# Chang-Tun-Yu/HLS-final-Visual-Odometry

Measured on AMD Instinct MI355X. Metric: stereo frame-pairs/sec (detect+match), KITTI 1241x376; matches bit-exact, higher is better.
Workload: dtype u8; 1 GPU; KITTI 1241x376 stereo quad-match (prev/curr x L/R), default 50x50 bins; noise=0, gpu_max_hw_queues=4, streams_per_gpu=256, frames_in_hbm=8, parallelism=1x independent stream groups

## Files before the change

### hls-final-visual-odometry_amd/csrc/kernels_match.hip

```cpp
#include "vh_findmatch.h"
#include "vh_wave.h"
#include <algorithm>
#include <cstdlib>
#include <type_traits>

#ifdef VH_FLOW_STATS
__device__ unsigned long long g_flow_stats[12];
extern "C" int32_t vh_debug_flow_stats(unsigned long long *out, int32_t reset) {
  if (hipMemcpyFromSymbol(out, HIP_SYMBOL(g_flow_stats), sizeof(g_flow_stats)) != hipSuccess) return -3;
  if (reset) { unsigned long long z[12] = {0}; if (hipMemcpyToSymbol(HIP_SYMBOL(g_flow_stats), z, sizeof(z)) != hipSuccess) return -3; }
  return 0;
}
#define VH_STAT(k, n) do { if ((threadIdx.x & 63) == 0) atomicAdd(&g_flow_stats[k], (unsigned long long)(n)); } while (0)
#else
#define VH_STAT(k, n) do { } while (0)
#endif

#ifndef VH_MATCH_WAVES
#define VH_MATCH_WAVES 7
#endif

namespace {

template <bool MAX>
__device__ __forceinline__ int32_t row16_allreduce(int32_t v) {
#define VH_ROW_STEP(CTRL)                                                                   \
  {                                                                                         \
    const int32_t t = __builtin_amdgcn_update_dpp(v, v, CTRL, 0xF, 0xF, false);             \
    v = MAX ? max(v, t) : min(v, t);                                                        \
  }
  VH_ROW_STEP(0x128)
  VH_ROW_STEP(0x124)
  VH_ROW_STEP(0x122)
  VH_ROW_STEP(0x121)
#undef VH_ROW_STEP
  return v;
}

template <class T>
__device__ __forceinline__ T ld_off(const T *base, uint32_t byte_off) { return *(const T *)((const char *)base + byte_off); }
template <class T>
__device__ __forceinline__ void st_off(T *base, uint32_t byte_off, T x) { *(T *)((char *)base + byte_off) = x; }
template <class T>
__device__ __forceinline__ T ld_uniform(const T *p) { return *(const __attribute__((address_space(4))) T *)(uintptr_t)p; }
__device__ __forceinline__ int32_t ld_uniform_i32(const int32_t *p) { return __builtin_amdgcn_readfirstlane(ld_uniform(p)); }

template <bool TESTED, class First, class Step>
__device__ __forceinline__ void walk_columns(const VhSets &s, const int32_t *__restrict__ cbs, int32_t c, int32_t UB0, int32_t UB1, int32_t VB0,
                                             int32_t VB1, int32_t ULO_MAX, int32_t UHI_MIN, int32_t VA0, int32_t VA1, First first, Step step) {
  const int32_t lane = threadIdx.x & 63;
  const bool merged = !TESTED && VB0 == 0 && VB1 == s.vbn - 1;
  const int32_t UB1w = merged ? UB0 : UB1;
  for (int32_t cb = UB0; cb <= UB1w; cb += 64) {
    const int32_t ncb = min(64, UB1w - cb + 1);
    int32_t t_p0 = 0, t_p1 = 0, t_a0 = 0, t_a1 = 0;
    if (lane < ncb) {
      const int32_t row = (c * s.ubn + cb + lane) * s.vbn;
      t_p0 = ld_off(cbs, (uint32_t)(row + VB0) * 4u);
      t_p1 = ld_off(cbs, (uint32_t)(merged ? (c * s.ubn + UB1 + 1) * s.vbn : row + VB1 + 1) * 4u);
      if (TESTED) {
        const int32_t ubx = cb + lane;
        const bool in_ = ubx * s.binsize >= ULO_MAX && ubx * s.binsize + s.binsize - 1 <= UHI_MIN;
        t_a0 = in_ ? ((VA0 <= VA1) ? cbs[row + VA0] : t_p1) : 1;
        t_a1 = in_ ? ((VA0 <= VA1) ? cbs[row + VA1 + 1] : t_p1) : 0;
      }
    }
    int32_t ci = -1, pc = -64, p1 = 0;
    const auto advance = [&]() -> bool {
      pc += 64;
      while (pc >= p1) {
        if (++ci >= ncb) return false;
        pc = __builtin_amdgcn_readlane(t_p0, ci); p1 = __builtin_amdgcn_readlane(t_p1, ci);
      }
      return true;
    };
    if (!advance()) continue;
    first(pc, p1);
    for (;;) {
      const int32_t c_pc = pc, c_p1 = p1, c_ci = ci;
      const bool more = advance();
      int32_t pa0 = 1, pa1 = 0;
      if (TESTED) { pa0 = __builtin_amdgcn_readlane(t_a0, c_ci); pa1 = __builtin_amdgcn_readlane(t_a1, c_ci); }
      step(c_pc, c_p1, pa0, pa1, more, pc, p1);
      if (!more) break;
    }
  }
}

template <bool TESTED, bool NEED_UV, class Consume>
__device__ __forceinline__ void walk_region(const VhSets &s, const int32_t *__restrict__ cbs, const uint32_t *__restrict__ cuv,
                                            const uint4 *__restrict__ cdesc, int32_t c, int32_t UB0, int32_t UB1, int32_t VB0,
                                            int32_t VB1, int32_t ULO_MAX, int32_t UHI_MIN, int32_t VA0, int32_t VA1,
                                            Consume consume) {
  const int32_t lane = threadIdx.x & 63;
  int32_t pl = 0;
  uint32_t gu = 0;
  uint4 g0, g1;
  const auto load = [&](int32_t pc, int32_t p1) __attribute__((always_inline)) {
    pl = min(pc + lane, p1 - 1);
    if (NEED_UV) gu = cuv[pl];
    g0 = cdesc[2 * (int64_t)pl]; g1 = cdesc[2 * (int64_t)pl + 1];
  };
  walk_columns<TESTED>(s, cbs, c, UB0, UB1, VB0, VB1, ULO_MAX, UHI_MIN, VA0, VA1, load,
    [&](int32_t pc, int32_t p1, int32_t pa0, int32_t pa1, bool more, int32_t npc, int32_t np1) __attribute__((always_inline)) {
      const int32_t c_pl = pl;
      const uint32_t c_gu = gu;
      const uint4 c_g0 = g0, c_g1 = g1;
      if (more) load(npc, np1);
      consume(pc, p1, pa0, pa1, c_pl, c_gu, c_g0, c_g1);
    });
}

__device__ __forceinline__ void glds16(const void *gbase, uint32_t byte_off, uint32_t lds_dst) {
  asm volatile("s_mov_b32 m0, %2\n\ts_nop 0\n\tglobal_load_lds_dwordx4 %0, %1" ::"v"(byte_off), "s"(gbase), "s"(lds_dst) : "memory");
}
__device__ __forceinline__ void glds4(const void *gbase, uint32_t byte_off, uint32_t lds_dst) {
  asm volatile("s_mov_b32 m0, %2\n\ts_nop 0\n\tglobal_load_lds_dword %0, %1" ::"v"(byte_off), "s"(gbase), "s"(lds_dst) : "memory");
}
__device__ __forceinline__ uint32_t lds_addr(const void *p) {
  return __builtin_amdgcn_readfirstlane((uint32_t)(uintptr_t)(const __attribute__((address_space(3))) void *)p);
}

template <bool TESTED, class Consume>
__device__ __forceinline__ void walk_region_lds(const VhSets &s, const int32_t *__restrict__ cbs, const uint32_t *__restrict__ cuv,
                                                const uint4 *__restrict__ cdesc, int32_t c, int32_t UB0, int32_t UB1, int32_t VB0,
                                                int32_t VB1, int32_t ULO_MAX, int32_t UHI_MIN, int32_t VA0, int32_t VA1,
                                                uint4 *wD, uint32_t *wU, Consume consume) {
  const uint32_t ldsD = lds_addr(wD), ldsU = lds_addr(wU);
  const uint32_t lane32 = (uint32_t)(threadIdx.x & 63) * 32u;
  const auto issue = [&](int32_t b, int32_t pc, int32_t p1) __attribute__((always_inline)) {
    const uint32_t off = min((uint32_t)pc * 32u + lane32, (uint32_t)(p1 - 1) * 32u);
    glds16(cdesc, off, ldsD + (uint32_t)b * 2048u); glds16(cdesc, off + 16u, ldsD + (uint32_t)b * 2048u + 1024u);
    if (TESTED) glds4(cuv, off >> 3, ldsU + (uint32_t)b * 256u);
  };
  int32_t buf = 0;
  walk_columns<TESTED>(s, cbs, c, UB0, UB1, VB0, VB1, ULO_MAX, UHI_MIN, VA0, VA1,
    [&](int32_t pc, int32_t p1) __attribute__((always_inline)) {
      asm volatile("s_waitcnt lgkmcnt(0)" ::: "memory");
      buf = 0;
      issue(0, pc, p1);
    },
    [&](int32_t pc, int32_t p1, int32_t pa0, int32_t pa1, bool more, int32_t npc, int32_t np1) __attribute__((always_inline)) {
      const int32_t c_buf = buf;
      if (more) {
        buf ^= 1;
        asm volatile("s_waitcnt lgkmcnt(0)" ::: "memory");
        issue(buf, npc, np1);
        if (TESTED) asm volatile("s_waitcnt vmcnt(3)" ::: "memory");
        else asm volatile("s_waitcnt vmcnt(2)" ::: "memory");
      } else {
        asm volatile("s_waitcnt vmcnt(0)" ::: "memory");
      }
      consume(pc, p1, pa0, pa1, (const uint4 *)(wD + c_buf * 128), (const uint32_t *)(wU + c_buf * 64));
    });
}

__device__ __forceinline__ uint64_t tested_key_uniform_query(const uint32_t (&qd)[8], us2 lo2, us2 span2, uint32_t uv2,
                                                             const uint4 &b0, const uint4 &b1, uint32_t relpos) {
  const bool out = outside_window(uv2, lo2, span2);
  const uint32_t sad = sad32(make_uint4(qd[0], qd[1], qd[2], qd[3]), make_uint4(qd[4], qd[5], qd[6], qd[7]), b0, b1, 0);
  return out ? ~0ull : (((uint64_t)sad << 32) | relpos);
}

enum { KEY_HI16 = 0, KEY_W19 = 1, KEY_64 = 2 };
template <int KM> struct KeyT { typedef uint32_t type; };
template <> struct KeyT<KEY_64> { typedef uint64_t type; };
template <int KM>
__device__ __forceinline__ typename KeyT<KM>::type sad_key(const uint4 &a0, const uint4 &a1, const uint4 &b0, const uint4 &b1, uint32_t seed) {
  if (KM == KEY_HI16) return (typename KeyT<KM>::type)sad32<true>(a0, a1, b0, b1, seed);
  const uint32_t sad = sad32(a0, a1, b0, b1, 0);
  if (KM == KEY_W19) return (typename KeyT<KM>::type)((sad << 19) | seed);
  return (typename KeyT<KM>::type)(((uint64_t)sad << 32) | seed);
}
template <int KM>
__device__ __forceinline__ typename KeyT<KM>::type key_none_floor() {
  typedef typename KeyT<KM>::type key_t;
  return KM == KEY_HI16 ? (key_t)0xFFFF0000u : KM == KEY_W19 ? (key_t)0xFFF80000u : (key_t)0x0000FFFF00000000ull;
}
__device__ __forceinline__ int32_t key_mode_of(int32_t class_count, int32_t wide_keys) {
  if (class_count + 64 <= 0x10000 && !wide_keys) return KEY_HI16;
  return class_count <= VH_CLASS_POS_MAX && wide_keys < 2 ? KEY_W19 : KEY_64;
}

template <int Q, int P, int KM>
__device__ __forceinline__ int32_t join_phases(const typename KeyT<KM>::type (&best_key)[Q]) {
  static_assert(Q == 2 && P == 4, "the join splits the wave into two slots of two 16-lane rows");
  if (KM == KEY_64) {
    uint64_t k[Q];
#pragma unroll
    for (int32_t qi = 0; qi < Q; qi++) {
      k[qi] = (uint64_t)best_key[qi];
#pragma unroll
      for (int32_t d = 16; d < 64; d <<= 1) k[qi] = min(k[qi], vh_shfl_xor_u64(k[qi], d));
    }
    const uint64_t kk = (threadIdx.x & 32) ? k[1] : k[0];
    return kk >= key_none_floor<KEY_64>() ? -1 : (int32_t)(uint32_t)kk;
  }
  const auto h = __builtin_amdgcn_permlane32_swap((uint32_t)best_key[0], (uint32_t)best_key[1], false, false);
  const uint32_t kh = min(h[0], h[1]);
  const auto r = __builtin_amdgcn_permlane16_swap(kh, kh, false, false);
  const uint32_t k = min(r[0], r[1]);
  return k >= key_none_floor<KM>() ? -1 : (int32_t)(k & (KM == KEY_HI16 ? 0xFFFFu : 0x7FFFFu));
}

#ifndef VH_REDO_G
#define VH_REDO_G 2
#endif
struct RedoGroup {
  uint32_t qd[VH_REDO_G][8];
  us2 lo2[VH_REDO_G];
  int32_t lane[VH_REDO_G], n;
  int32_t umin, umax, vmin, vmax;
};
template <int Q>
__device__ __forceinline__ bool redo_take(uint64_t &todo, const uint4 (&a0)[Q], const uint4 (&a1)[Q], const uint32_t (&uv1)[Q],
                                          int32_t radius, int32_t rv, RedoGroup &g) {
  g.n = 0; g.umin = g.vmin = 0x7FFFFFFF; g.umax = g.vmax = -1;
#pragma unroll
  for (int32_t k = 0; k < VH_REDO_G; k++) {
    if (!todo) break;
    const int32_t fl = (int32_t)__builtin_ctzll(todo), fq = fl >> 5;
    todo &= todo - 1;
    uint4 x0 = a0[0], x1 = a1[0];
    uint32_t xu = uv1[0];
#pragma unroll
    for (int32_t qi = 1; qi < Q; qi++) if (fq == qi) { x0 = a0[qi]; x1 = a1[qi]; xu = uv1[qi]; }
    g.qd[k][0] = __builtin_amdgcn_readlane(x0.x, fl); g.qd[k][1] = __builtin_amdgcn_readlane(x0.y, fl);
    g.qd[k][2] = __builtin_amdgcn_readlane(x0.z, fl); g.qd[k][3] = __builtin_amdgcn_readlane(x0.w, fl);
    g.qd[k][4] = __builtin_amdgcn_readlane(x1.x, fl); g.qd[k][5] = __builtin_amdgcn_readlane(x1.y, fl);
    g.qd[k][6] = __builtin_amdgcn_readlane(x1.z, fl); g.qd[k][7] = __builtin_amdgcn_readlane(x1.w, fl);
    const uint32_t quv1 = __builtin_amdgcn_readlane(xu, fl);
    const int32_t u1 = (int32_t)(quv1 & 0xFFFF), v1 = (int32_t)(quv1 >> 16);
    g.lo2[k] = window_lo2(quv1, radius, rv);
    g.lane[k] = fl; g.n = k + 1;
    g.umin = min(g.umin, u1); g.umax = max(g.umax, u1); g.vmin = min(g.vmin, v1); g.vmax = max(g.vmax, v1);
  }
  return g.n > 0;
}

template <int Q> struct TileOut {
  int32_t wp;
  uint4 a0[Q], a1[Q];
  uint32_t uv1[Q];
  int32_t qpos[Q];
  bool valid[Q];
};

template <int Q, int P, bool SPEC, bool FLOW>
__device__ __forceinline__ void finish_tile(const VhSets &s, const VhMatchArgs &a, int32_t pass, int32_t stream, int32_t qset, int32_t cset,
                                            int32_t c, int32_t pbase, int32_t pcnt, const TileOut<Q> &o,
                                            int32_t *__restrict__ best, int32_t *__restrict__ redo_count) {
  static_assert(Q == 2 && P == 4, "one query per lane: slot lane >> 5, on the first 16-lane row of each half (join_phases)");
  const int32_t lane = threadIdx.x & 63;
  const uint32_t *__restrict__ cuv = s.s_uv + (int64_t)cset * s.cap;
  const uint4 *__restrict__ cdesc = (const uint4 *)(s.s_desc + (int64_t)cset * s.cap * 8);
  const int32_t *__restrict__ cbs = s.bin_start + (int64_t)cset * (s.nbins + 1);
  const int32_t rv = FLOW ? a.radius : a.disp_tol;
  const us2 span2 = window_span2(a.radius, rv);
  const int32_t *__restrict__ cidx = s.s_idx + (int64_t)cset * s.cap;
  const int32_t *__restrict__ qidx = s.s_idx + (int64_t)qset * s.cap;
  int32_t *__restrict__ tbl = best + ((int64_t)stream * 4 + a.pass[pass].slot) * s.cap;
  const bool hi = lane & 32;
  const bool mine = !(lane & 16) && (hi ? o.valid[1] : o.valid[0]);
  const uint32_t uv1 = hi ? o.uv1[1] : o.uv1[0];
  const int32_t qpos = hi ? o.qpos[1] : o.qpos[0];
  int32_t res = -1;
  bool fail = false;
  if (mine && o.wp >= 0) {
    int32_t wp = o.wp;
    VH_CHECK_RANGE(s, 7, wp, 0, pcnt);
    res = pbase + wp;
    if (SPEC) fail = outside_window(ld_off(cuv, (uint32_t)res * 4u), window_lo2(uv1, a.radius, rv), span2);
  }
  if (SPEC) {
    uint64_t todo = __ballot(fail);
    if (todo) {
      const int32_t nfail = (int32_t)__popcll(todo);
      VH_STAT(FLOW ? 7 : 10, nfail);
      if (lane == 0) atomicAdd(redo_count, nfail);
      RedoGroup g;
      while (redo_take<Q>(todo, o.a0, o.a1, o.uv1, a.radius, rv, g)) {
        uint64_t kk[VH_REDO_G];
#pragma unroll
        for (int32_t k = 0; k < VH_REDO_G; k++) kk[k] = ~0ull;
        if (FLOW) {
          const VhBins b = bins_of_interest(s, VhWindow{g.umin - a.radius, g.umax + a.radius, g.vmin - rv, g.vmax + rv});
          walk_region<false, true>(s, cbs, cuv, cdesc, c, b.ub0, b.ub1, b.vb0, b.vb1, 0, 0, 0, 0,
            [&](int32_t, int32_t, int32_t, int32_t, int32_t pl, uint32_t gu, const uint4 &g0, const uint4 &g1) {
#pragma unroll
              for (int32_t k = 0; k < VH_REDO_G; k++)
                if (k < g.n) kk[k] = min(kk[k], tested_key_uniform_query(g.qd[k], g.lo2[k], span2, gu, g0, g1, (uint32_t)(pl - pbase)));
            });
        } else {
          const int32_t *__restrict__ crs = s.row_start + (int64_t)cset * (4 * s.H + 1);
          const int32_t *__restrict__ cpos = s.r_pos + (int64_t)cset * s.cap;
          const int32_t x0 = ld_uniform_i32(crs + c * s.H + max(g.vmin - rv, 0));
          const int32_t x1 = ld_uniform_i32(crs + c * s.H + min(g.vmax + rv, s.H - 1) + 1);
          for (int32_t x = x0 + lane; x < x1; x += 64) {
            int32_t cp = cpos[x];
            VH_CHECK_RANGE(s, 3, cp, pbase, pbase + pcnt);
            const uint32_t gu = cuv[cp];
            const uint4 g0 = cdesc[2 * (int64_t)cp], g1 = cdesc[2 * (int64_t)cp + 1];
#pragma unroll
            for (int32_t k = 0; k < VH_REDO_G; k++)
              if (k < g.n) kk[k] = min(kk[k], tested_key_uniform_query(g.qd[k], g.lo2[k], span2, gu, g0, g1, (uint32_t)(cp - pbase)));
          }
        }
#pragma unroll
        for (int32_t k = 0; k < VH_REDO_G; k++)
          if (k < g.n) {
            const uint64_t kf = vh_wave_min_u64(kk[k]);
            int32_t wp = (int32_t)(uint32_t)kf;
            if (kf != ~0ull) VH_CHECK_RANGE(s, 7, wp, 0, pcnt);
            if (lane == g.lane[k]) res = kf == ~0ull ? -1 : pbase + wp;
          }
      }
    }
  }
  if (mine) st_off(tbl, (uint32_t)ld_off(qidx, (uint32_t)qpos * 4u) * 4u, res < 0 ? 0 : ld_off(cidx, (uint32_t)res * 4u));
}

struct FlowRegion {
  int32_t UB0, UB1, VB0, VB1;
  int32_t ULO_MAX, UHI_MIN, VA0, VA1;
};
template <int Q, int P, bool SPEC>
__device__ __forceinline__ FlowRegion flow_queries(const VhSets &s, const VhMatchArgs &a, int32_t rv, int32_t qset, int32_t q0, int32_t q1,
                                                   int32_t c, TileOut<Q> &out) {
  constexpr int L = 64 / P;
  static_assert(L == 8 || L == 16, "every 16-lane row must hold the whole tile (row-wise window reduction)");
  const int32_t l = (threadIdx.x & 63) % L;
  const uint32_t *__restrict__ quv = s.s_uv + (int64_t)qset * s.cap;
  const uint4 *__restrict__ qdesc = (const uint4 *)(s.s_desc + (int64_t)qset * s.cap * 8);
  bool (&valid)[Q] = out.valid;
  uint4 (&a0)[Q] = out.a0, (&a1)[Q] = out.a1;
  uint32_t (&uv1)[Q] = out.uv1;
  int32_t umin = 0x7FFFFFFF, umax = -1, vmin = 0x7FFFFFFF, vmax = -1;
  int32_t (&qp)[Q] = out.qpos;
  const int32_t *__restrict__ qsnake = s.snake_pos + (int64_t)qset * s.cap;
#pragma unroll
  for (int32_t qi = 0; qi < Q; qi++) {
    const int32_t q = q0 + L * qi + l;
    valid[qi] = q < q1;
    qp[qi] = valid[qi] ? q : q0;
    if (VH_SNAKE) qp[qi] = ld_off(qsnake, (uint32_t)qp[qi] * 4u);
#ifdef VH_CHECK
    {
      const int32_t *qbs = s.bin_start + (int64_t)qset * (s.nbins + 1);
      VH_CHECK_RANGE(s, 14, qp[qi], qbs[c * s.ubn * s.vbn], qbs[(c + 1) * s.ubn * s.vbn]);
    }
#endif
  }
#pragma unroll
  for (int32_t qi = 0; qi < Q; qi++) {
    const int32_t ql = qp[qi];
    uv1[qi] = ld_off(quv, (uint32_t)ql * 4u);
    a0[qi] = ld_off(qdesc, (uint32_t)ql * 32u); a1[qi] = ld_off(qdesc, (uint32_t)ql * 32u + 16u);
    const int32_t u1 = uv1[qi] & 0xFFFF, v1 = uv1[qi] >> 16;
    umin = min(umin, u1); umax = max(umax, u1); vmin = min(vmin, v1); vmax = max(vmax, v1);
  }
  umin = __builtin_amdgcn_readfirstlane(row16_allreduce<false>(umin));
  umax = __builtin_amdgcn_readfirstlane(row16_allreduce<true>(umax));
  vmin = __builtin_amdgcn_readfirstlane(row16_allreduce<false>(vmin));
  vmax = __builtin_amdgcn_readfirstlane(row16_allreduce<true>(vmax));
  const VhBins ub = bins_of_interest(s, VhWindow{umin - a.radius, umax + a.radius, vmin - rv, vmax + rv});
  FlowRegion r;
  r.UB0 = ub.ub0; r.UB1 = ub.ub1; r.VB0 = ub.vb0; r.VB1 = ub.vb1;
  r.ULO_MAX = umax - a.radius; r.UHI_MIN = umin + a.radius;
  const int32_t VLO_MAX = vmax - rv, VHI_MIN = vmin + rv;
  r.VA0 = SPEC ? 0 : max(r.VB0, (max(VLO_MAX, 0) + s.binsize - 1) / s.binsize);
  r.VA1 = SPEC ? 0 : min(r.VB1, (VHI_MIN + 1) / s.binsize - 1);
  VH_STAT(0, 1); VH_STAT(5, q1 - q0); VH_STAT(6, r.UB1 - r.UB0 + 1);
  return r;
}

template <int Q, int P, int KM, bool SPEC>
__device__ __forceinline__ void flow_tile(const VhSets &s, const VhMatchArgs &a, int32_t rv, int32_t cset, int32_t c, const FlowRegion &r,
                                          int32_t pbase, uint4 *wD, uint32_t *wU, TileOut<Q> &out) {
  constexpr int L = 64 / P;
  constexpr int TRIP = 2 * P;
  constexpr int CH = 64 / TRIP;
  static_assert(P * (2 * CH - 1) <= 64, "the chunk-local seeds P * k must be inline constants (integers up to 64)");
  const int32_t ph = (threadIdx.x & 63) / L;
  const uint32_t *__restrict__ cuv = s.s_uv + (int64_t)cset * s.cap;
  const uint4 *__restrict__ cdesc = (const uint4 *)(s.s_desc + (int64_t)cset * s.cap * 8);
  const int32_t *__restrict__ cbs = s.bin_start + (int64_t)cset * (s.nbins + 1);
  const uint4 (&a0)[Q] = out.a0, (&a1)[Q] = out.a1;
  typedef typename KeyT<KM>::type key_t;
  const key_t KNONE = (key_t)~(key_t)0;
  key_t best_key[Q];
  int32_t v_lo[Q];
  us2 lo2[Q];
#pragma unroll
  for (int32_t qi = 0; qi < Q; qi++) {
    v_lo[qi] = (int32_t)(out.uv1[qi] >> 16) - rv;
    lo2[qi] = window_lo2(out.uv1[qi], a.radius, rv);
    best_key[qi] = KNONE;
  }
  const us2 span2 = window_span2(a.radius, rv);

  constexpr uint32_t LNONE = 0xFFFF0000u;
  auto make_key = [&](auto test, int32_t qi, uint32_t uv2, const uint4 &b0, const uint4 &b1, uint32_t seed) -> uint32_t {
    constexpr int TEST = decltype(test)::value;
    bool out = false;
    if (TEST == 2) {
      out = outside_window(uv2, lo2[qi], span2);
    } else if (TEST == 1) {
      out = (uint32_t)((int32_t)(uv2 >> 16) - v_lo[qi]) > (uint32_t)(2 * rv);
    }
    const uint32_t key = sad_key<KEY_HI16>(a0[qi], a1[qi], b0, b1, seed);
    return (TEST != 0 && out) ? LNONE : key;
  };
  auto global_key = [](uint32_t k, uint32_t vbase) -> key_t {
    if (KM == KEY_HI16) return (key_t)(k + vbase);
    const uint32_t pos = (k & 0xFFFFu) + vbase;
    if (KM == KEY_W19) return (key_t)(((k & 0xFFFF0000u) << 3) | pos);
    return (key_t)(((uint64_t)(k >> 16) << 32) | pos);
  };
  walk_region_lds<!SPEC>(s, cbs, cuv, cdesc, c, r.UB0, r.UB1, r.VB0, r.VB1, r.ULO_MAX, r.UHI_MIN, r.VA0, r.VA1, wD, wU,
    [&](int32_t pc, int32_t p1, int32_t pa0, int32_t pa1, const uint4 *cD, const uint32_t *cU) {
      VH_STAT(1, 1);
      const int32_t mcnt = min(64, p1 - pc);
      const int32_t nt = (mcnt + TRIP - 1) / TRIP;
      const uint4 *rd = cD + ph;
      const uint32_t *ru = cU + ph;
      uint32_t cm[Q];
      auto trip = [&](auto test, int32_t t) __attribute__((always_inline)) {
        VH_STAT(2 + decltype(test)::value, 1);
        const int32_t o = TRIP * t;
        const uint4 dA0 = rd[o], dA1 = rd[o + 64], dB0 = rd[o + P], dB1 = rd[o + 64 + P];
        uint32_t uA = 0, uB = 0;
        if (decltype(test)::value != 0) { uA = ru[o]; uB = ru[o + P]; }
#pragma unroll
        for (int32_t qi = 0; qi < Q; qi++) {
          const uint32_t kA = make_key(test, qi, uA, dA0, dA1, (uint32_t)o), kB = make_key(test, qi, uB, dB0, dB1, (uint32_t)(o + P));
          cm[qi] = t == 0 ? min(kA, kB) : min(min(kA, kB), cm[qi]);
        }
      };
      if (SPEC && nt == CH) {
#pragma unroll
        for (int32_t t = 0; t < CH; t++) {
          trip(std::integral_constant<int, 0>{}, t);
          if (t & 1) __builtin_amdgcn_sched_barrier(0);
        }
      } else if (SPEC || pa0 > pa1) {
        constexpr int TEST = SPEC ? 0 : 2;
#pragma unroll
        for (int32_t t = 0; t < CH; t++) {
          if (t >= nt) break;
          trip(std::integral_constant<int, TEST>{}, t);
        }
      } else {
        const int32_t ta = min((min(max(pa0 - pc, 0), mcnt) + TRIP - 1) / TRIP, nt);
        const int32_t tb = max(min(max(pa1 - pc, 0), mcnt) / TRIP, ta);
#pragma unroll
        for (int32_t t = 0; t < CH; t++) {
          if (t >= nt) break;
          if (t >= ta && t < tb) trip(std::integral_constant<int, 0>{}, t);
          else trip(std::integral_constant<int, 1>{}, t);
        }
      }
      const uint32_t vbase = (uint32_t)(pc - pbase + ph);
#pragma unroll
      for (int32_t qi = 0; qi < Q; qi++) best_key[qi] = min(best_key[qi], global_key(cm[qi], vbase));
    });
  out.wp = join_phases<Q, P, KM>(best_key);
}

template <bool SPEC, bool FLOW, class Tile>
__device__ __forceinline__ void search_tile(const VhSets &s, const VhMatchArgs &a, int32_t pass, int32_t stream, int32_t qset, int32_t cset,
                                            int32_t c, int32_t *__restrict__ best, int32_t *__restrict__ redo_count,
                                            TileOut<VH_FLOW_Q> &out, Tile tile) {
  const int32_t *cbs = s.bin_start + (int64_t)cset * (s.nbins + 1);
  const int32_t pbase = ld_uniform_i32(cbs + c * s.ubn * s.vbn);
  const int32_t pend = ld_uniform_i32(cbs + (c + 1) * s.ubn * s.vbn);
  const int32_t km = key_mode_of(pend - pbase, a.wide_keys);
  if (km == KEY_HI16) tile(std::integral_constant<int, KEY_HI16>{}, pbase, pend - pbase);
  else if (km == KEY_W19) tile(std::integral_constant<int, KEY_W19>{}, pbase, pend - pbase);
  else tile(std::integral_constant<int, KEY_64>{}, pbase, pend - pbase);
  finish_tile<VH_FLOW_Q, VH_FLOW_P, SPEC, FLOW>(s, a, pass, stream, qset, cset, c, pbase, pend - pbase, out, best, redo_count);
}

template <bool SPEC>
__device__ __forceinline__ void flow_pass(const VhSets &s, const VhMatchArgs &a, int32_t pass, int32_t stream, int32_t qset,
                                          int32_t cset, uint4 *wD, uint32_t *wU, int32_t *__restrict__ best, int32_t *__restrict__ redo_count) {
  const int32_t ntile = ld_uniform_i32(s.tile_cnt + qset);
  for (int32_t tile = __builtin_amdgcn_readfirstlane(blockIdx.x * 4 + (threadIdx.x >> 6)); tile < ntile;
       tile += gridDim.x * 4) {
    typedef int32_t i32x4 __attribute__((ext_vector_type(4)));
    const i32x4 t = ld_uniform((const i32x4 *)(s.tiles + (int64_t)qset * s.max_tiles + tile));
    const int32_t q0 = __builtin_amdgcn_readfirstlane(t.x), q1 = __builtin_amdgcn_readfirstlane(t.y);
    const int32_t c = __builtin_amdgcn_readfirstlane(t.z);
    TileOut<VH_FLOW_Q> out;
    const int32_t rv = a.pass[pass].flow ? a.radius : a.disp_tol;
    const FlowRegion r = flow_queries<VH_FLOW_Q, VH_FLOW_P, SPEC>(s, a, rv, qset, q0, q1, c, out);
    search_tile<SPEC, true>(s, a, pass, stream, qset, cset, c, best, redo_count, out,
      [&](auto km, int32_t pbase, int32_t) __attribute__((always_inline)) {
        flow_tile<VH_FLOW_Q, VH_FLOW_P, decltype(km)::value, SPEC>(s, a, rv, cset, c, r, pbase, wD, wU, out);
      });
  }
}

template <int Q, int P, int KM, bool SPEC>
__device__ __forceinline__ void rows_tile(const VhSets &s, const VhMatchArgs &a, int32_t pass, int32_t stream, int32_t qset,
                                          int32_t cset, int32_t q0, int32_t q1, int32_t c, int32_t pbase, int32_t pcnt, uint4 *wD,
                                          uint32_t *wU, uint32_t *wV, TileOut<Q> &out) {
  constexpr int L = 64 / P;
  static_assert(L == 8 || L == 16, "every 16-lane row must hold the whole tile");
  constexpr int TRIP = 2 * P;
  const int32_t lane = threadIdx.x & 63, ph = lane / L, l = lane % L;
  const int32_t nrow = 4 * s.H;
  const int32_t *__restrict__ crs = s.row_start + (int64_t)cset * (nrow + 1);
  const int32_t *__restrict__ qpos = s.r_pos + (int64_t)qset * s.cap;
  const uint32_t *__restrict__ quv = s.s_uv + (int64_t)qset * s.cap;
  const uint4 *__restrict__ qdesc = (const uint4 *)(s.s_desc + (int64_t)qset * s.cap * 8);
  const int32_t *__restrict__ cpos = s.r_pos + (int64_t)cset * s.cap;
  const uint32_t *__restrict__ cuv = s.s_uv + (int64_t)cset * s.cap;
  const uint4 *__restrict__ cdesc = (const uint4 *)(s.s_desc + (int64_t)cset * s.cap * 8);

  bool (&valid)[Q] = out.valid;
  uint4 (&a0)[Q] = out.a0, (&a1)[Q] = out.a1;
  uint32_t (&uv1)[Q] = out.uv1;
  int32_t (&qp)[Q] = out.qpos;
  typedef typename KeyT<KM>::type key_t;
  key_t best_key[Q];
  us2 lo2[Q];
  const us2 span2 = window_span2(a.radius, a.disp_tol);
  int32_t vmin = 0x7FFFFFFF, vmax = -1;
#pragma unroll
  for (int32_t qi = 0; qi < Q; qi++) {
    const int32_t q = q0 + L * qi + l;
    valid[qi] = q < q1;
    qp[qi] = ld_off(qpos, (uint32_t)(valid[qi] ? q : q0) * 4u);
    VH_CHECK_RANGE(s, 1, qp[qi], 0, s.cap);
    uv1[qi] = ld_off(quv, (uint32_t)qp[qi] * 4u);
    a0[qi] = ld_off(qdesc, (uint32_t)qp[qi] * 32u); a1[qi] = ld_off(qdesc, (uint32_t)qp[qi] * 32u + 16u);
    const int32_t v1 = uv1[qi] >> 16;
    lo2[qi] = window_lo2(uv1[qi], a.radius, a.disp_tol);
    best_key[qi] = (key_t)~(key_t)0;
    vmin = min(vmin, v1); vmax = max(vmax, v1);
  }
  vmin = __builtin_amdgcn_readfirstlane(row16_allreduce<false>(vmin));
  vmax = __builtin_amdgcn_readfirstlane(row16_allreduce<true>(vmax));
  VH_STAT(8, 1); VH_STAT(11, q1 - q0);
  const int32_t VLO = max(vmin - a.disp_tol, 0), VHI = min(vmax + a.disp_tol, s.H - 1);
  const int32_t r0 = ld_uniform_i32(crs + c * s.H + VLO);
  const int32_t r1 = ld_uniform_i32(crs + c * s.H + VHI + 1);
  for (int32_t rc = r0; rc < r1; rc += 64) {
    const int32_t mcnt = min(64, r1 - rc);
    int32_t cp = ld_off(cpos, (uint32_t)min(rc + lane, r1 - 1) * 4u);
    VH_CHECK_RANGE(s, 2, cp, pbase, pbase + pcnt);
    const uint4 g0 = ld_off(cdesc, (uint32_t)cp * 32u), g1 = ld_off(cdesc, (uint32_t)cp * 32u + 16u);
    uint32_t gu = 0;
    if (!SPEC) gu = ld_off(cuv, (uint32_t)cp * 4u);
    asm volatile("s_waitcnt lgkmcnt(0)" ::: "memory");
    wD[lane] = g0; wD[64 + lane] = g1; wU[lane] = (uint32_t)(cp - pbase);
    if (!SPEC) wV[lane] = gu;
    asm volatile("s_waitcnt lgkmcnt(0)" ::: "memory");
    const int32_t jend = (mcnt + TRIP - 1) & ~(TRIP - 1);
    VH_STAT(9, jend / TRIP);
    const uint4 *rd = wD + ph;
    const uint32_t *ru = wU + ph, *rv = wV + ph;
    for (int32_t j = 0; j < jend; j += TRIP) {
      const uint4 dA0 = rd[0], dA1 = rd[64], dB0 = rd[P], dB1 = rd[64 + P];
      const uint32_t sA = ru[0], sB = ru[P];
      uint32_t uA = 0, uB = 0;
      if (!SPEC) { uA = rv[0]; uB = rv[P]; }
#pragma unroll
      for (int32_t qi = 0; qi < Q; qi++) {
        key_t kA = sad_key<KM>(a0[qi], a1[qi], dA0, dA1, sA), kB = sad_key<KM>(a0[qi], a1[qi], dB0, dB1, sB);
        if (!SPEC) {
          kA = outside_window(uA, lo2[qi], span2) ? (key_t)~(key_t)0 : kA;
          kB = outside_window(uB, lo2[qi], span2) ? (key_t)~(key_t)0 : kB;
        }
        best_key[qi] = min(min(kA, kB), best_key[qi]);
      }
      rd += TRIP; ru += TRIP; rv += TRIP;
    }
  }
  out.wp = join_phases<Q, P, KM>(best_key);
}

template <bool SPEC>
__device__ __forceinline__ void rows_pass(const VhSets &s, const VhMatchArgs &a, int32_t pass, int32_t stream, int32_t qset,
                                          int32_t cset, uint4 *wD, uint32_t *wU, uint32_t *wV, int32_t *__restrict__ best, int32_t *__restrict__ redo_count) {
  const int32_t nrow = 4 * s.H;
  const int32_t *__restrict__ qrs = s.row_start + (int64_t)qset * (nrow + 1);
  int32_t cls_q0[5];
#pragma unroll
  for (int32_t c = 0; c <= 4; c++) cls_q0[c] = ld_uniform_i32(qrs + c * s.H);
  constexpr int T = VH_TILE_Q;
  for (int32_t tile = __builtin_amdgcn_readfirstlane(blockIdx.x * 4 + (threadIdx.x >> 6));; tile += gridDim.x * 4) {
    int32_t c = -1, q0 = 0, q1 = 0, t = tile;
#pragma unroll
    for (int32_t k = 0; k < 4; k++) {
      const int32_t nt = (cls_q0[k + 1] - cls_q0[k] + T - 1) / T;
      if (c < 0 && t < nt) { c = k; q0 = cls_q0[k] + T * t; q1 = min(cls_q0[k + 1], q0 + T); }
      if (c < 0) t -= nt;
    }
    if (c < 0) break;
    TileOut<VH_FLOW_Q> out;
    search_tile<SPEC, false>(s, a, pass, stream, qset, cset, c, best, redo_count, out,
      [&](auto km, int32_t pbase, int32_t pcnt) __attribute__((always_inline)) {
        rows_tile<VH_FLOW_Q, VH_FLOW_P, decltype(km)::value, SPEC>(s, a, pass, stream, qset, cset, q0, q1, c, pbase, pcnt, wD, wU, wV, out);
      });
  }
}

template <bool SPEC>
__global__ void __launch_bounds__(256) __attribute__((amdgpu_waves_per_eu(VH_MATCH_WAVES, 8)))
match_kernel(VhSets s, VhMatchArgs a, int32_t *__restrict__ best, int32_t *__restrict__ redo) {
  __shared__ uint4 sDesc[4 * 256];
  __shared__ uint32_t sAux[4 * 128];
  __shared__ uint32_t sAux2[SPEC ? 1 : 4 * 64];
  const int32_t pass = blockIdx.y, stream = blockIdx.z;
  if (a.prior && pass == 1) return;
#ifdef VH_EXP_SKIP
  if (VH_EXP_SKIP & (a.pass[pass].flow ? 2 : 1)) return;
#endif
  const int32_t qset = vh_row_set(a, stream, a.pass[pass].qset);
  const int32_t cset = vh_row_set(a, stream, a.pass[pass].cset);
  uint4 *wD = sDesc + (threadIdx.x >> 6) * 256;
  uint32_t *wU = sAux + (threadIdx.x >> 6) * 128;
  uint32_t *wV = sAux2 + (SPEC ? 0 : (threadIdx.x >> 6) * 64);
  int32_t *redo_count = redo + stream;
  if (a.pass[pass].flow) flow_pass<SPEC>(s, a, pass, stream, qset, cset, wD, wU, best, redo_count);
  else rows_pass<SPEC>(s, a, pass, stream, qset, cset, wD, wU, wV, best, redo_count);
}

}

void vh_launch_match(const VhSets &s, const VhMatchArgs &a, int32_t *best, int32_t *redo, int32_t speculative, int32_t grid_x,
                     int32_t lds_bytes, hipStream_t st) {
  if (!a.npass) return;
  VhMatchArgs m = a;
  static const int wide = [] { const char *e = getenv("VH_FLOW_WIDE_KEYS"); return e ? atoi(e) : 0; }();
  m.wide_keys = wide;
  static const int wgs = [] { const char *e = getenv("VH_FLOW_WGS"); return e ? atoi(e) : 0; }();
  static const int pad_env = [] { const char *e = getenv("VH_FLOW_LDS_PAD"); return e ? atoi(e) : -1; }();
  const int32_t gx = wgs > 0 ? wgs : (grid_x > 0 ? (grid_x | 1) : (((s.max_tiles + 3) / 4) | 1));
  dim3 grid(gx, m.npass, a.rows);
  static const size_t static_lds[2] = {
      [] { hipFuncAttributes at{}; return hipFuncGetAttributes(&at, (const void *)match_kernel<false>) == hipSuccess ? at.sharedSizeBytes : (size_t)0; }(),
      [] { hipFuncAttributes at{}; return hipFuncGetAttributes(&at, (const void *)match_kernel<true>) == hipSuccess ? at.sharedSizeBytes : (size_t)0; }()};
  const size_t have = static_lds[speculative ? 1 : 0];
  const int32_t pad = pad_env >= 0 ? pad_env : (wgs > 0 || grid_x <= 0 || lds_bytes <= 0 || have == 0 || (size_t)lds_bytes <= have ? 0 : (int32_t)((size_t)lds_bytes - have));
  if (speculative) hipLaunchKernelGGL(match_kernel<true>, grid, dim3(256), pad, st, s, m, best, redo);
  else hipLaunchKernelGGL(match_kernel<false>, grid, dim3(256), pad, st, s, m, best, redo);
}
```

Baseline: 120,800 pairs/s.

## Prefetch candidate positions, unroll row-match chunks, and simplify tile bookkeeping

Reworks the stereo rows matching tile. The next chunk's candidate position load is issued early so its latency overlaps the current chunk's SAD work. The inner trip loop is fully unrolled with sched barriers for full 64-candidate chunks. The row vmin/vmax comes from the first and last query instead of a DPP allreduce, which relies on queries being sorted by row. Per-query valid flags become a query count turned into a lane mask via inverse ballot, and tile-to-class lookup uses precomputed prefix tile counts. These changes add unrolled code size and register pressure, and depend on the sort-order assumption holding.

```diff
diff --git a/hls-final-visual-odometry_amd/csrc/kernels_match.hip b/hls-final-visual-odometry_amd/csrc/kernels_match.hip
--- a/hls-final-visual-odometry_amd/csrc/kernels_match.hip
+++ b/hls-final-visual-odometry_amd/csrc/kernels_match.hip
@@ -26,7 +26,7 @@
 __device__ __forceinline__ int32_t row16_allreduce(int32_t v) {
 #define VH_ROW_STEP(CTRL)                                                                   \
   {                                                                                         \
-    const int32_t t = __builtin_amdgcn_update_dpp(v, v, CTRL, 0xF, 0xF, false);             \
+    const int32_t t = __builtin_amdgcn_update_dpp(0, v, CTRL, 0xF, 0xF, true);              \
     v = MAX ? max(v, t) : min(v, t);                                                        \
   }
   VH_ROW_STEP(0x128)
@@ -243,7 +243,7 @@
   uint4 a0[Q], a1[Q];
   uint32_t uv1[Q];
   int32_t qpos[Q];
-  bool valid[Q];
+  int32_t nq;
 };
 
 template <int Q, int P, bool SPEC, bool FLOW>
@@ -261,7 +261,8 @@
   const int32_t *__restrict__ qidx = s.s_idx + (int64_t)qset * s.cap;
   int32_t *__restrict__ tbl = best + ((int64_t)stream * 4 + a.pass[pass].slot) * s.cap;
   const bool hi = lane & 32;
-  const bool mine = !(lane & 16) && (hi ? o.valid[1] : o.valid[0]);
+  const uint64_t owners = ((1ull << min(o.nq, 16)) - 1ull) | (((1ull << max(o.nq - 16, 0)) - 1ull) << 32);
+  const bool mine = __builtin_amdgcn_inverse_ballot_w64(owners);
   const uint32_t uv1 = hi ? o.uv1[1] : o.uv1[0];
   const int32_t qpos = hi ? o.qpos[1] : o.qpos[0];
   int32_t res = -1;
@@ -332,7 +333,8 @@
   const int32_t l = (threadIdx.x & 63) % L;
   const uint32_t *__restrict__ quv = s.s_uv + (int64_t)qset * s.cap;
   const uint4 *__restrict__ qdesc = (const uint4 *)(s.s_desc + (int64_t)qset * s.cap * 8);
-  bool (&valid)[Q] = out.valid;
+  bool valid[Q];
+  out.nq = q1 - q0;
   uint4 (&a0)[Q] = out.a0, (&a1)[Q] = out.a1;
   uint32_t (&uv1)[Q] = out.uv1;
   int32_t umin = 0x7FFFFFFF, umax = -1, vmin = 0x7FFFFFFF, vmax = -1;
@@ -508,6 +510,7 @@
   constexpr int L = 64 / P;
   static_assert(L == 8 || L == 16, "every 16-lane row must hold the whole tile");
   constexpr int TRIP = 2 * P;
+  constexpr int CH = 64 / TRIP;
   const int32_t lane = threadIdx.x & 63, ph = lane / L, l = lane % L;
   const int32_t nrow = 4 * s.H;
   const int32_t *__restrict__ crs = s.row_start + (int64_t)cset * (nrow + 1);
@@ -518,7 +521,6 @@
   const uint32_t *__restrict__ cuv = s.s_uv + (int64_t)cset * s.cap;
   const uint4 *__restrict__ cdesc = (const uint4 *)(s.s_desc + (int64_t)cset * s.cap * 8);
 
-  bool (&valid)[Q] = out.valid;
   uint4 (&a0)[Q] = out.a0, (&a1)[Q] = out.a1;
   uint32_t (&uv1)[Q] = out.uv1;
   int32_t (&qp)[Q] = out.qpos;
@@ -526,57 +528,78 @@
   key_t best_key[Q];
   us2 lo2[Q];
   const us2 span2 = window_span2(a.radius, a.disp_tol);
-  int32_t vmin = 0x7FFFFFFF, vmax = -1;
+  out.nq = q1 - q0;
+  const uint32_t lane4 = (uint32_t)lane * 4u;
 #pragma unroll
   for (int32_t qi = 0; qi < Q; qi++) {
-    const int32_t q = q0 + L * qi + l;
-    valid[qi] = q < q1;
-    qp[qi] = ld_off(qpos, (uint32_t)(valid[qi] ? q : q0) * 4u);
+    qp[qi] = ld_off(qpos, min((uint32_t)(q0 + L * qi) * 4u + (uint32_t)l * 4u, (uint32_t)(q1 - 1) * 4u));
     VH_CHECK_RANGE(s, 1, qp[qi], 0, s.cap);
     uv1[qi] = ld_off(quv, (uint32_t)qp[qi] * 4u);
     a0[qi] = ld_off(qdesc, (uint32_t)qp[qi] * 32u); a1[qi] = ld_off(qdesc, (uint32_t)qp[qi] * 32u + 16u);
-    const int32_t v1 = uv1[qi] >> 16;
     lo2[qi] = window_lo2(uv1[qi], a.radius, a.disp_tol);
     best_key[qi] = (key_t)~(key_t)0;
-    vmin = min(vmin, v1); vmax = max(vmax, v1);
-  }
-  vmin = __builtin_amdgcn_readfirstlane(row16_allreduce<false>(vmin));
-  vmax = __builtin_amdgcn_readfirstlane(row16_allreduce<true>(vmax));
+  }
+  const int32_t vmin = (int32_t)(__builtin_amdgcn_readlane(uv1[0], 0) >> 16);
+  const int32_t vmax = (int32_t)(__builtin_amdgcn_readlane(uv1[Q - 1], L - 1) >> 16);
+#ifdef VH_CHECK
+#pragma unroll
+  for (int32_t qi = 0; qi < Q; qi++) { int32_t v1 = (int32_t)(uv1[qi] >> 16); VH_CHECK_RANGE(s, 15, v1, vmin, vmax + 1); }
+#endif
   VH_STAT(8, 1); VH_STAT(11, q1 - q0);
   const int32_t VLO = max(vmin - a.disp_tol, 0), VHI = min(vmax + a.disp_tol, s.H - 1);
   const int32_t r0 = ld_uniform_i32(crs + c * s.H + VLO);
   const int32_t r1 = ld_uniform_i32(crs + c * s.H + VHI + 1);
+  const auto position_of = [&](int32_t rc) __attribute__((always_inline)) {
+    return ld_off(cpos, min((uint32_t)rc * 4u + lane4, (uint32_t)(r1 - 1) * 4u));
+  };
+  const uint4 *rd = wD + ph;
+  const uint32_t *ru = wU + ph, *rv = wV + ph;
+  auto trip = [&](int32_t t) __attribute__((always_inline)) {
+    const int32_t o = TRIP * t;
+    const uint4 dA0 = rd[o], dA1 = rd[o + 64], dB0 = rd[o + P], dB1 = rd[o + 64 + P];
+    const uint32_t sA = ru[o], sB = ru[o + P];
+    uint32_t uA = 0, uB = 0;
+    if (!SPEC) { uA = rv[o]; uB = rv[o + P]; }
+#pragma unroll
+    for (int32_t qi = 0; qi < Q; qi++) {
+      key_t kA = sad_key<KM>(a0[qi], a1[qi], dA0, dA1, sA), kB = sad_key<KM>(a0[qi], a1[qi], dB0, dB1, sB);
+      if (!SPEC) {
+        kA = outside_window(uA, lo2[qi], span2) ? (key_t)~(key_t)0 : kA;
+        kB = outside_window(uB, lo2[qi], span2) ? (key_t)~(key_t)0 : kB;
+      }
+      best_key[qi] = min(min(kA, kB), best_key[qi]);
+    }
+  };
+  int32_t cp = 0;
+  if (r0 < r1) cp = position_of(r0);
   for (int32_t rc = r0; rc < r1; rc += 64) {
     const int32_t mcnt = min(64, r1 - rc);
-    int32_t cp = ld_off(cpos, (uint32_t)min(rc + lane, r1 - 1) * 4u);
     VH_CHECK_RANGE(s, 2, cp, pbase, pbase + pcnt);
     const uint4 g0 = ld_off(cdesc, (uint32_t)cp * 32u), g1 = ld_off(cdesc, (uint32_t)cp * 32u + 16u);
     uint32_t gu = 0;
     if (!SPEC) gu = ld_off(cuv, (uint32_t)cp * 4u);
-    asm volatile("s_waitcnt lgkmcnt(0)" ::: "memory");
-    wD[lane] = g0; wD[64 + lane] = g1; wU[lane] = (uint32_t)(cp - pbase);
+    const uint32_t seed = (uint32_t)(cp - pbase);
+    if (SPEC && rc + 64 < r1) cp = position_of(rc + 64);
+    asm volatile("" ::: "memory");
+    wD[lane] = g0; wD[64 + lane] = g1; wU[lane] = seed;
     if (!SPEC) wV[lane] = gu;
     asm volatile("s_waitcnt lgkmcnt(0)" ::: "memory");
-    const int32_t jend = (mcnt + TRIP - 1) & ~(TRIP - 1);
-    VH_STAT(9, jend / TRIP);
-    const uint4 *rd = wD + ph;
-    const uint32_t *ru = wU + ph, *rv = wV + ph;
-    for (int32_t j = 0; j < jend; j += TRIP) {
-      const uint4 dA0 = rd[0], dA1 = rd[64], dB0 = rd[P], dB1 = rd[64 + P];
-      const uint32_t sA = ru[0], sB = ru[P];
-      uint32_t uA = 0, uB = 0;
-      if (!SPEC) { uA = rv[0]; uB = rv[P]; }
-#pragma unroll
-      for (int32_t qi = 0; qi < Q; qi++) {
-        key_t kA = sad_key<KM>(a0[qi], a1[qi], dA0, dA1, sA), kB = sad_key<KM>(a0[qi], a1[qi], dB0, dB1, sB);
-        if (!SPEC) {
-          kA = outside_window(uA, lo2[qi], span2) ? (key_t)~(key_t)0 : kA;
-          kB = outside_window(uB, lo2[qi], span2) ? (key_t)~(key_t)0 : kB;
-        }
-        best_key[qi] = min(min(kA, kB), best_key[qi]);
-      }
-      rd += TRIP; ru += TRIP; rv += TRIP;
-    }
+    const int32_t nt = (mcnt + TRIP - 1) / TRIP;
+    VH_STAT(9, nt);
+    if (nt == CH) {
+#pragma unroll
+      for (int32_t t = 0; t < CH; t++) {
+        trip(t);
+        if (t & 1) __builtin_amdgcn_sched_barrier(0);
+      }
+    } else {
+#pragma unroll
+      for (int32_t t = 0; t < CH; t++) {
+        if (t >= nt) break;
+        trip(t);
+      }
+    }
+    if (!SPEC && rc + 64 < r1) cp = position_of(rc + 64);
   }
   out.wp = join_phases<Q, P, KM>(best_key);
 }
@@ -586,19 +609,19 @@
                                           int32_t cset, uint4 *wD, uint32_t *wU, uint32_t *wV, int32_t *__restrict__ best, int32_t *__restrict__ redo_count) {
   const int32_t nrow = 4 * s.H;
   const int32_t *__restrict__ qrs = s.row_start + (int64_t)qset * (nrow + 1);
-  int32_t cls_q0[5];
+  constexpr int T = VH_TILE_Q;
+  int32_t cls_q0[5], cls_t0[5];
 #pragma unroll
   for (int32_t c = 0; c <= 4; c++) cls_q0[c] = ld_uniform_i32(qrs + c * s.H);
-  constexpr int T = VH_TILE_Q;
-  for (int32_t tile = __builtin_amdgcn_readfirstlane(blockIdx.x * 4 + (threadIdx.x >> 6));; tile += gridDim.x * 4) {
-    int32_t c = -1, q0 = 0, q1 = 0, t = tile;
-#pragma unroll
-    for (int32_t k = 0; k < 4; k++) {
-      const int32_t nt = (cls_q0[k + 1] - cls_q0[k] + T - 1) / T;
-      if (c < 0 && t < nt) { c = k; q0 = cls_q0[k] + T * t; q1 = min(cls_q0[k + 1], q0 + T); }
-      if (c < 0) t -= nt;
-    }
-    if (c < 0) break;
+  cls_t0[0] = 0;
+#pragma unroll
+  for (int32_t c = 0; c < 4; c++) cls_t0[c + 1] = cls_t0[c] + (int32_t)((uint32_t)(cls_q0[c + 1] - cls_q0[c] + T - 1) / (uint32_t)T);
+  for (int32_t tile = __builtin_amdgcn_readfirstlane(blockIdx.x * 4 + (threadIdx.x >> 6)); tile < cls_t0[4]; tile += gridDim.x * 4) {
+    int32_t c = 0, tb = 0, qb = cls_q0[0], qe = cls_q0[1];
+#pragma unroll
+    for (int32_t k = 1; k < 4; k++)
+      if (tile >= cls_t0[k]) { c = k; tb = cls_t0[k]; qb = cls_q0[k]; qe = cls_q0[k + 1]; }
+    const int32_t q0 = qb + T * (tile - tb), q1 = min(qe, q0 + T);
     TileOut<VH_FLOW_Q> out;
     search_tile<SPEC, false>(s, a, pass, stream, qset, cset, c, best, redo_count, out,
       [&](auto km, int32_t pbase, int32_t pcnt) __attribute__((always_inline)) {
```

Result: no change. 121,400 pairs/s, median of 6 (+0.5%).
